# khwajamoiz01/cadence

Hardware: AMD Instinct MI355X
Metric: history events replayed/sec (node) + workflows rebuilt/sec; % HBM peak (higher is better)
Workload: dtype int64

## Files before the change

cadence_amd/csrc/replay_kernel.hip:

```cpp

#include <hip/hip_runtime.h>
#include <stddef.h>
#include <stdint.h>

#include <type_traits>
#include <utility>

#include "cadence_replay.h"

#ifndef CRR_LDS_ACT
#define CRR_LDS_ACT 2
#endif
#ifndef CRR_LDS_TIMER
#define CRR_LDS_TIMER 2
#endif
#ifndef CRR_LDS_CHILD
#define CRR_LDS_CHILD 1
#endif
#ifndef CRR_LDS_RC
#define CRR_LDS_RC 1
#endif
#ifndef CRR_LDS_SIG
#define CRR_LDS_SIG 1
#endif
// ... 2570 lines not shown
    i64 bt = 0, be = 0;
    if (cnt > CRR_WAVE_MIN_SCALAR) {
      i64 v = 0x7fffffffffffffffLL;
      each<N>([&](auto k) { v = (ok[k] && t[k] < v) ? t[k] : v; });
      const i64 wm = WaveTables<HbmRows>::wave_min_i64(v);
      each<N>([&](auto k) { m[k] = __builtin_amdgcn_ballot_w64(ok[k] && t[k] == wm); });
    }
    each<N>([&](auto k) {
      for (u64 x = m[k]; x; x &= x - 1) {
        const i32 l = (i32)__builtin_ctzll(x);
        const i64 tt = readlane_i64(t[k], l), ee = readlane_i64(id[k], l);
        if (best < 0 || tt < bt || (tt == bt && ee < be)) { best = 64 * k + l; bt = tt; be = ee; }
      }
    });
    tmin = bt;
    return best;
  }
  __device__ __forceinline__ void epilogue(Lane& L, const Geo& G, const TaskSink& K) {
    if (L.n_act > 0 && dirty_act) {
      u32 ok[NA];
      each<NA>([&](auto k) { ok[k] = (a_fl[k] & (kMirLive | kMirHave)) == (kMirLive | kMirHave); });
      i64 t = 0;
      const i32 j = argmin<NA>(ok, a_ct, a_id, t);
      if (j >= 0) {
        const u32 fl = get<NA>(a_fl, j);
        const i32 y = (i32)((fl >> 9) & 7u);
        if (!(fl & kMirCreated)) {
          set_bits<NA>(a_fl, j, kMirCreated | (timer_mask(y) << 16), 0u);
          if (y == CRR_TIMEOUT_HEARTBEAT) M->act[j].last_hb_timeout_vis_s = unix_seconds(t);
          if (K.on) K.add(L, G, CRR_TASK_ACTIVITY_TIMEOUT, y, L.current_version, t, get<NA>(a_id, j), M->act[j].attempt, -1);
        }
      }
    }
    dirty_act = false;
    if (L.n_timer > 0 && dirty_timer) {
      u32 ok[NT];
      each<NT>([&](auto k) { ok[k] = (t_fl[k] & kMirLive) != 0; });
      i64 t = 0;
      const i32 j = argmin<NT>(ok, t_ex, t_sid, t);
      if (j >= 0 && !(get<NT>(t_fl, j) & kMirTimerCreated)) {
        set_bits<NT>(t_fl, j, kMirTimerCreated, 0u);
        K.add(L, G, CRR_TASK_USER_TIMER, 0, L.current_version, t, get<NT>(t_sid, j), 0, -1);
      }
    }
    dirty_timer = false;
  }
  __device__ __forceinline__ void refresh(Lane& L, const Geo& G) {
    each<NA>([&](auto k) { a_fl[k] &= ~(kMirCreated | (0xffu << 16)); });
    each<NT>([&](auto k) { t_fl[k] &= ~kMirTimerCreated; });
    dirty_act = dirty_timer = true;
    epilogue(L, G, TaskSink{false, false});
  }

  template <int N, class Row, class Patch>
  __device__ __forceinline__ void scatter(const u32 (&fl)[N], const i64 (&id)[N], Row* rows, i64* ids,
                                          Row* (Geo::*dst)(i32) const, const Geo& G, Patch patch) const {
    i32 rank[N];
    u64 live[N];
    each<N>([&](auto k) { rank[k] = 0; live[k] = __builtin_amdgcn_ballot_w64((fl[k] & kMirLive) != 0); });
    each<N>([&](auto k2) {
      for (u64 x = live[k2]; x; x &= x - 1) {
        const i64 o = readlane_i64(id[k2], (i32)__builtin_ctzll(x));
        each<N>([&](auto k) { rank[k] += o < id[k] ? 1 : 0; });
      }
    });
    each<N>([&](auto k) {
      if ((fl[k] & kMirLive) != 0) {
        Row r = rows[64 * k + lane];
        patch(r, fl[k]);
        *(G.*dst)(rank[k]) = r;
        ids[rank[k]] = id[k];
      }
    });
  }
  __device__ __forceinline__ void finalize(Lane& L, const Geo& G) {
    i64* ids = M->ids;
    constexpr i32 oT = A, oC = oT + T, oR = oC + C, oS = oR + R;
    scatter<NA>(a_fl, a_id, M->act, ids, &Geo::act, G, [](crr_activity_row& r, u32 f) {
      r.flags = f & 0xffu;
      r.timer_task_status = (i32)((f >> 16) & 0xffu);
    });
    scatter<NT>(t_fl, t_sid, M->timer, ids + oT, &Geo::timer, G, [](crr_timer_row& r, u32 f) {
      r.flags = f & 0xffu;
      r.task_status = (f & kMirTimerCreated) ? CRR_TIMER_TASK_STATUS_CREATED : CRR_TIMER_TASK_STATUS_NONE;
    });
    scatter<NC>(c_fl, c_id, M->child, ids + oC, &Geo::child, G, [](crr_child_row& r, u32 f) { r.flags = f & 0xffu; });
    scatter<NR>(r_fl, r_id, M->rc, ids + oR, &Geo::rc, G, [](crr_initiated_row& r, u32 f) { r.flags = f & 0xffu; });
    scatter<NS>(s_fl, s_id, M->sig, ids + oS, &Geo::sig, G, [](crr_initiated_row& r, u32 f) { r.flags = f & 0xffu; });
    if (lane < L.n_rp) *G.rp(lane) = M->rp[lane];
    wave_sync_lds();
  }
  __device__ __forceinline__ i64 act_id(const Geo&, i32 i) const { return M->ids[i]; }
  __device__ __forceinline__ i64 timer_id(const Geo&, i32 i) const { return M->ids[A + i]; }
  __device__ __forceinline__ i64 child_id(const Geo&, i32 i) const { return M->ids[A + T + i]; }
  __device__ __forceinline__ i64 rc_id(const Geo&, i32 i) const { return M->ids[A + T + C + i]; }
  __device__ __forceinline__ i64 sig_id(const Geo&, i32 i) const { return M->ids[A + T + C + R + i]; }
  __device__ __forceinline__ void retry_push(const crr_inputs& in, const crr_outputs& out, u32 w) {
    retried = true;
    if constexpr (kList >= 0) {
      if (lane == 0) {
        const u32 k = atomicAdd(out.scratch + kList, 1u);
        out.scratch[retry_slot(in, kList, k)] = w;
      }
    }
  }
};

#if CRR_WAVE_REG
template <class ARENA, int LIST>
using WaveLds = WaveRegTables<ARENA, LIST>;
template <class ARENA, int LIST>
__device__ __forceinline__ void bind_arena(WaveRegTables<ARENA, LIST>& T, ARENA* a) { T.M = a; }
#else
template <class ARENA, int LIST>
using WaveLds = WaveTables<LdsRows<ARENA, LIST>>;
template <class ARENA, int LIST>
__device__ __forceinline__ void bind_arena(WaveTables<LdsRows<ARENA, LIST>>& T, ARENA* a) { T.S.M = a; }
#endif


namespace need {
constexpr u64 bit(int t) { return 1ull << t; }
constexpr u64 kTs = bit(CRR_EV_DECISION_TASK_SCHEDULED) | bit(CRR_EV_DECISION_TASK_STARTED) |
                    bit(CRR_EV_ACTIVITY_TASK_SCHEDULED) | bit(CRR_EV_ACTIVITY_TASK_STARTED) | bit(CRR_EV_TIMER_STARTED);
constexpr u64 kRef = bit(CRR_EV_DECISION_TASK_SCHEDULED) | bit(CRR_EV_DECISION_TASK_STARTED) |
                     bit(CRR_EV_DECISION_TASK_COMPLETED) | bit(CRR_EV_ACTIVITY_TASK_STARTED) |
                     bit(CRR_EV_ACTIVITY_TASK_COMPLETED) | bit(CRR_EV_ACTIVITY_TASK_FAILED) |
                     bit(CRR_EV_ACTIVITY_TASK_TIMED_OUT) | bit(CRR_EV_ACTIVITY_TASK_CANCELED) | bit(CRR_EV_TIMER_STARTED) |
                     bit(CRR_EV_START_CHILD_WORKFLOW_EXECUTION_FAILED) | bit(CRR_EV_CHILD_WORKFLOW_EXECUTION_STARTED) |
                     bit(CRR_EV_CHILD_WORKFLOW_EXECUTION_COMPLETED) | bit(CRR_EV_CHILD_WORKFLOW_EXECUTION_FAILED) |
                     bit(CRR_EV_CHILD_WORKFLOW_EXECUTION_CANCELED) | bit(CRR_EV_CHILD_WORKFLOW_EXECUTION_TIMED_OUT) |
                     bit(CRR_EV_CHILD_WORKFLOW_EXECUTION_TERMINATED) | bit(CRR_EV_REQUEST_CANCEL_EXTERNAL_FAILED) |
                     bit(CRR_EV_EXTERNAL_WORKFLOW_EXECUTION_CANCEL_REQUESTED) | bit(CRR_EV_SIGNAL_EXTERNAL_FAILED) |
                     bit(CRR_EV_EXTERNAL_WORKFLOW_EXECUTION_SIGNALED);
constexpr u64 kKey = bit(CRR_EV_DECISION_TASK_COMPLETED) | bit(CRR_EV_ACTIVITY_TASK_SCHEDULED) |
                     bit(CRR_EV_ACTIVITY_TASK_CANCEL_REQUESTED) | bit(CRR_EV_TIMER_STARTED) | bit(CRR_EV_TIMER_FIRED) |
                     bit(CRR_EV_TIMER_CANCELED);
constexpr u64 kAux = bit(CRR_EV_WORKFLOW_EXECUTION_STARTED) | bit(CRR_EV_DECISION_TASK_SCHEDULED) |
                     bit(CRR_EV_ACTIVITY_TASK_SCHEDULED) | bit(CRR_EV_REQUEST_CANCEL_EXTERNAL_INITIATED) |
                     bit(CRR_EV_WORKFLOW_EXECUTION_CONTINUED_AS_NEW) |
                     bit(CRR_EV_START_CHILD_WORKFLOW_EXECUTION_INITIATED) | bit(CRR_EV_SIGNAL_EXTERNAL_INITIATED);
constexpr u64 kTsTasks = bit(CRR_EV_WORKFLOW_EXECUTION_STARTED) | bit(CRR_EV_WORKFLOW_EXECUTION_COMPLETED) |
                         bit(CRR_EV_WORKFLOW_EXECUTION_FAILED) | bit(CRR_EV_WORKFLOW_EXECUTION_TIMED_OUT) |
                         bit(CRR_EV_WORKFLOW_EXECUTION_CANCELED) | bit(CRR_EV_WORKFLOW_EXECUTION_TERMINATED) |
                         bit(CRR_EV_WORKFLOW_EXECUTION_CONTINUED_AS_NEW);
__device__ __forceinline__ bool has(u64 mask, u32 et) { return (mask >> (et & CRR_ETYPE_MASK)) & 1ull; }
}

struct LaneSource {
  const crr_events& E;
  i64 begin, st;
  i32 n;
  Ev nx;
  u32 et_nx;
  u64 ts_mask;
  u64 aux_mask;
  __device__ __forceinline__ LaneSource(const crr_events& e, i64 b, i64 stride, i32 count, bool tasks, bool started_aux = false)
      : E(e), begin(b), st(stride), n(count), ts_mask(need::kTs | (tasks ? need::kTsTasks : 0ull)),
        aux_mask(need::kAux | (started_aux ? need::bit(CRR_EV_ACTIVITY_TASK_STARTED) : 0ull)) {}
  __device__ __forceinline__ i64 ix(i32 step) const { return begin + (i64)step * st; }
  __device__ __forceinline__ Ev load(i32 step, u32 et) const {
    Ev e;
    const i64 i = ix(step);
    e.et = et;
    e.id_ = E.event_id[i];
    e.ver_ = E.version[i];
    e.ts_ = need::has(ts_mask, et) ? E.timestamp[i] : 0;
    e.ref_ = need::has(need::kRef, et) ? E.ref[i] : 0;
    e.key_ = need::has(need::kKey, et) ? E.key[i] : 0u;
    e.aux_ = need::has(aux_mask, et) ? E.aux[i] : 0;
    e.task_ = 0;
    return e;
  }
  __device__ __forceinline__ void start() {
    if (n > 0) {
      const i64 i = ix(0);
      nx.et = E.etype[i];
      et_nx = E.etype[ix(n > 1 ? 1 : 0)];
      nx.id_ = E.event_id[i];
      nx.ver_ = E.version[i];
      nx.ts_ = E.timestamp[i];
      nx.ref_ = E.ref[i];
      nx.key_ = E.key[i];
      nx.aux_ = E.aux[i];
      nx.task_ = 0;
    }
  }
  __device__ __forceinline__ Ev next(i32 s) {
    const Ev e = nx;
    issue(s);
    return e;
  }
  __device__ __forceinline__ void issue(i32 s) {
    if (s + 1 < n) nx = load(s + 1, et_nx);
    if (s + 2 < n) et_nx = E.etype[ix(s + 2)];
  }
  __device__ __forceinline__ i64 task_id(i32 step) const { return E.task_id[ix(step)]; }
};

struct WaveLaneSource : LaneSource {
  i64 ubase;
  __device__ __forceinline__ WaveLaneSource(const crr_events& e, i64 b, i32 count, bool tasks)
      : LaneSource(e, b, 64, count, tasks), ubase(uniform64(b - (i64)threadIdx.x)) {}
  template <class T>
  __device__ __forceinline__ T at(const T* col, i32 step) const {
    static_assert(sizeof(T) == 1 || sizeof(T) == 4 || sizeof(T) == 8, "column width");
    const i64 row = uniform64((i64)reinterpret_cast<uintptr_t>(col + (ubase + (i64)step * 64)));
    u32 off;
    if constexpr (sizeof(T) == 1) asm("v_mov_b32 %0, %1 ; step %2" : "=v"(off) : "v"(threadIdx.x), "s"(step));
    else if constexpr (sizeof(T) == 4) asm("v_lshlrev_b32 %0, 2, %1 ; step %2" : "=v"(off) : "v"(threadIdx.x), "s"(step));
    else asm("v_lshlrev_b32 %0, 3, %1 ; step %2" : "=v"(off) : "v"(threadIdx.x), "s"(step));
    typedef const T __attribute__((address_space(1))) * global_ptr;
    return *(global_ptr)((u64)row + (u64)off);
  }
  __device__ __forceinline__ Ev load(i32 step, u32 et) const {
    Ev e;
    e.et = et;
    e.id_ = at(E.event_id, step);
    e.ver_ = at(E.version, step);
    e.ts_ = need::has(ts_mask, et) ? at(E.timestamp, step) : 0;
    e.ref_ = need::has(need::kRef, et) ? at(E.ref, step) : 0;
    e.key_ = need::has(need::kKey, et) ? at(E.key, step) : 0u;
    e.aux_ = need::has(aux_mask, et) ? at(E.aux, step) : 0;
    e.task_ = 0;
    return e;
  }
  __device__ __forceinline__ void start() {
    if (n > 0) {
      nx.et = at(E.etype, 0);
      et_nx = E.etype[ix(n > 1 ? 1 : 0)];
      nx.id_ = at(E.event_id, 0);
      nx.ver_ = at(E.version, 0);
      nx.ts_ = at(E.timestamp, 0);
      nx.ref_ = at(E.ref, 0);
      nx.key_ = at(E.key, 0);
      nx.aux_ = at(E.aux, 0);
      nx.task_ = 0;
    }
  }
  __device__ __forceinline__ Ev next(i32 s) {
    const Ev e = nx;
    issue(s);
    return e;
  }
  __device__ __forceinline__ void issue(i32 s) {
    const i32 su = uniform32(s);
    if (s + 1 < n) nx = load(su + 1, et_nx);
    if (s + 2 < n) et_nx = at(E.etype, su + 2);
  }
};

#ifndef CRR_WAVE_FIELDS
#define CRR_WAVE_FIELDS 1
#endif
struct WaveSource {
  const crr_events& E;
  i64 begin, st;
  i32 n, lane;
  Ev cur, nxt;
  __device__ __forceinline__ WaveSource(const crr_events& e, i64 b, i64 stride, i32 count)
      : E(e), begin(b), st(stride), n(uniform32(count)) {
    lane = (i32)(threadIdx.x & 63);
  }
  __device__ __forceinline__ Ev load_chunk(i32 c) const {
    Ev e;
    const i32 s = c * 64 + lane;
    const i64 ix = begin + (i64)(s < n ? s : 0) * st;
    e.et = E.etype[ix]; e.id_ = E.event_id[ix]; e.ver_ = E.version[ix]; e.ts_ = E.timestamp[ix];
    e.task_ = 0; e.ref_ = E.ref[ix]; e.key_ = E.key[ix]; e.aux_ = E.aux[ix];
    return e;
  }
  __device__ __forceinline__ i64 task_id(i32 step) const { return E.task_id[begin + (i64)step * st]; }
  __device__ __forceinline__ void start() {
    if (n > 0) cur = load_chunk(0);
  }
  __device__ __forceinline__ void rotate() { cur = nxt; }
  __device__ __forceinline__ void issue_next(i32 c) {
    if ((c + 1) * 64 < n) nxt = load_chunk(c + 1);
  }
};
__device__ __forceinline__ u32 lane_u32(u32 v, i32 l) {
#if CRR_WAVE_FIELDS == 0
  return (u32)__shfl((int)v, l, 64);
#else
  const u32 r = __builtin_amdgcn_readlane(v, l);
#if CRR_WAVE_FIELDS == 2
  u32 o;
  asm("v_mov_b32 %0, %1" : "=v"(o) : "s"(r));
  return o;
#else
  return r;
#endif
#endif
}
__device__ __forceinline__ i64 lane_i64(i64 v, i32 l) {
  const u32 lo = lane_u32((u32)(u64)v, l), hi = lane_u32((u32)((u64)v >> 32), l);
  return (i64)(((u64)hi << 32) | lo);
}
struct SidePf {
  i32 s2s, s2c, st2c, hb, retry, dom;
};
struct WaveEv {
  const Ev& C;
  i32 l;
  u32 et;
  const SidePf* sp;
  __device__ __forceinline__ crr_activity_side act_side(const crr_inputs&) const {
    crr_activity_side a{};
    a.schedule_to_start = (i32)lane_u32((u32)sp->s2s, l);
    a.schedule_to_close = (i32)lane_u32((u32)sp->s2c, l);
    a.start_to_close = (i32)lane_u32((u32)sp->st2c, l);
    a.heartbeat = (i32)lane_u32((u32)sp->hb, l);
    a.has_retry_policy = (i32)lane_u32((u32)sp->retry, l);
    a.domain_status = (i32)lane_u32((u32)sp->dom, l);
    return a;
  }
  __device__ __forceinline__ i64 id() const { return lane_i64(C.id_, l); }
  __device__ __forceinline__ i64 ver() const { return lane_i64(C.ver_, l); }
  __device__ __forceinline__ i64 ts() const { return lane_i64(C.ts_, l); }
  __device__ __forceinline__ i64 task() const { return 0; }
  __device__ __forceinline__ i64 ref() const { return lane_i64(C.ref_, l); }
  __device__ __forceinline__ u32 key() const { return lane_u32(C.key_, l); }
  __device__ __forceinline__ i32 aux() const { return (i32)lane_u32((u32)C.aux_, l); }
};

struct TokenDesc { u32 so, sl, fo, fl; };
__device__ __forceinline__ TokenDesc token_desc(const crr_workflow* wfp) {
  return TokenDesc{wfp->start_token_off, wfp->start_token_len, wfp->final_token_off, wfp->final_token_len};
}
struct TokenWords {
  static constexpr int kWords = 12;
  u64 w[kWords];
  u32 off, len, held;
  u32 raw;
  bool spliced;
  __device__ __forceinline__ void issue(const TokenDesc& d, i32 token_src, const uint8_t* arena,
                                        const uint32_t* token_crc = nullptr, u32 wi = 0) {
    off = 0; len = 0;
    if (token_src == 1) { off = d.so; len = d.sl; }
    if (token_src == 2) { off = d.fo; len = d.fl; }
    spliced = token_src == 1 && token_crc != nullptr && len == kSpliceBytes;
    raw = spliced ? token_crc[wi] : 0u;
    held = (off & 7u) || spliced ? 0u : (len & ~7u);
    held = held < 8u * kWords ? held : 8u * kWords;
    const u64* tw = reinterpret_cast<const u64*>(arena + off);
#pragma unroll
    for (int j = 0; j < kWords; ++j) w[j] = (8u * j + 8u <= held) ? tw[j] : 0ull;
  }
};

template <class IDS>
__device__ __forceinline__ u32 payload_crc(const crr_exec_row& R, const IDS& ids, const Geo& G, const TokenWords& TW,
                                           const uint8_t* arena, const u32* tables, u32* out_len,
                                           bool have_last = false, i64 last_id = 0, i64 last_ver = 0,
                                           int64_t* const* sink = nullptr, bool sink_writer = false) {
  Crc K;
  K.init(tables);
  K.u8(0x59);
  K.field(2, 10); K.u8((R.flags & CRR_EXEC_CANCEL_REQUESTED) ? 1 : 0);
  K.field(6, 15); K.be16((u32)(uint16_t)(int16_t)R.state);
  K.field(10, 23); K.be64(R.last_first_event_id);
  K.field(10, 24); K.be64(R.next_event_id);
  K.field(10, 25); K.be64(R.last_processed_event);
  K.field(10, 26); K.be64((i64)R.signal_count);
  K.field(8, 35); K.be32((u32)(i32)R.decision_attempt);
  K.field(10, 36); K.be64(R.decision_version);
  K.field(10, 37); K.be64(R.decision_schedule_id);
  K.field(10, 38); K.be64(R.decision_started_id);
  const bool sk = sink != nullptr && sink_writer;
  auto put = [&](int t, i64 base, i32 i, i64 id) {
    if (sk) sink[t][base + (i64)i * G.st] = id;
    K.be64(id);
  };
  K.list_header(45, 10, (u32)R.n_timer);
  for (i32 i = 0; i < R.n_timer; ++i) put(1, G.timer_base, i, ids.timer_id(G, i));
  K.list_header(46, 10, (u32)R.n_activity);
  for (i32 i = 0; i < R.n_activity; ++i) put(0, G.act_base, i, ids.act_id(G, i));
  K.list_header(47, 10, (u32)R.n_signal);
  for (i32 i = 0; i < R.n_signal; ++i) put(4, G.sig_base, i, ids.sig_id(G, i));
  K.list_header(48, 10, (u32)R.n_rc);
  for (i32 i = 0; i < R.n_rc; ++i) put(3, G.rc_base, i, ids.rc_id(G, i));
  K.list_header(49, 10, (u32)R.n_child);
  for (i32 i = 0; i < R.n_child; ++i) put(2, G.child_base, i, ids.child_id(G, i));
  K.field(11, 55); K.be32(0);
  K.field(12, 56);
  K.field(8, 10); K.be32(0);
  K.list_header(20, 12, 1u);
  const u32 tlen = TW.len;
  K.field(11, 10); K.be32(tlen);
  if (TW.spliced) {
    K.splice(TW.raw);
  } else {
#pragma unroll
    for (int j = 0; j < TokenWords::kWords; ++j)
      if (8u * j + 8u <= TW.held) K.push(TW.w[j], 8);
    const uint8_t* tp = arena + TW.off;
    u32 i = TW.held;
    if ((TW.off & 7u) == 0) {
      const u64* tw = reinterpret_cast<const u64*>(tp);
      for (; i + 8 <= tlen; i += 8) K.push(tw[i >> 3], 8);
    }
// ... 704 lines not shown
        const u64 seg = le(lane) & ~le(bl);
        const bool carried_dirty = T.dirty_act || T.dirty_timer;
        u64 RPV = 0;
        for (u64 rpm = RP; rpm;) {
          const i32 j = (i32)__builtin_ctzll(rpm);
          const u32 key = __builtin_amdgcn_readlane(C.key_, j);
          rpm &= ~__builtin_amdgcn_ballot_w64(live && is_dc && C.key_ == key);
          if (!T.rp_has(L, G, key)) RPV |= 1ull << j;
        }
        const u64 EB = __builtin_amdgcn_ballot_w64(live && (C.et & CRR_ETYPE_BATCH_LAST) &&
                                                   ((MP & seg) != 0 || (bl < 0 && carried_dirty)));
        OPS = MP | RPV;
        vm = (OPS | EB) & le(stop - 1);
      }
      const u64 BF = __builtin_amdgcn_ballot_w64(live && (C.et & CRR_ETYPE_BATCH_FIRST));
      constexpr u64 kBatchIdTypes = (1ull << CRR_EV_ACTIVITY_TASK_SCHEDULED) |
                                    (1ull << CRR_EV_START_CHILD_WORKFLOW_EXECUTION_INITIATED) |
                                    (1ull << CRR_EV_REQUEST_CANCEL_EXTERNAL_INITIATED) |
                                    (1ull << CRR_EV_SIGNAL_EXTERNAL_INITIATED);
      i32 wfail = -1;
      int wrc = CRR_OK;
      while (vm) {
        const i32 j = (i32)__builtin_ctzll(vm);
        vm &= vm - 1;
        const i32 s = c0 + j;
        const WaveEv ev{C, j, (u32)__builtin_amdgcn_readlane(C.et, j), &SP};
        const u32 et = ev.et;
        i64 bfid = batch_first_id;
        if (!fast) {
          if (et & CRR_ETYPE_BATCH_FIRST) batch_first_id = ev.id();
          bfid = batch_first_id;
          L.current_version = L.state == CRR_STATE_COMPLETED ? lane_i64(pver, j) : ev.ver();
          last_task_step = s;
        } else if (((1ull << (et & CRR_ETYPE_MASK)) & kBatchIdTypes) != 0) {
          const i32 bf = last_in(BF & le(j));
          if (bf >= 0) bfid = lane_i64(C.id_, bf);
        }
        if (!fast || ((OPS >> j) & 1)) {
          const int rc = uniform32(apply_event(in, out, L, G, T, ev, s + L.src_base, (i32)(et & CRR_ETYPE_MASK), bfid,
                                               now_ns, K, retention_days));
          if (rc) {
            wfail = j;
            wrc = rc;
            break;
          }
        }
        if (et & CRR_ETYPE_BATCH_LAST) {
          T.epilogue(L, G, K);
          if (!fast) {
            L.last_first_event_id = batch_first_id;
            L.next_event_id = ev.id() + 1;
          }
        }
      }
      if (fast) {
        const i32 end = wfail >= 0 ? wfail : stop;
        const i32 dend = (wfail >= 0 && (__builtin_amdgcn_readlane(tl, wfail) == CRR_EV_DECISION_TASK_COMPLETED)) ? wfail + 1 : end;
        const bool lv = live && lane < dend;
        const bool is_ds = tl == CRR_EV_DECISION_TASK_SCHEDULED, is_dt = tl == CRR_EV_DECISION_TASK_STARTED;
        const bool is_dc = tl == CRR_EV_DECISION_TASK_COMPLETED;
        const bool is_df = tl == CRR_EV_DECISION_TASK_TIMED_OUT || tl == CRR_EV_DECISION_TASK_FAILED;
        const u64 DM = __builtin_amdgcn_ballot_w64(lv && (is_ds || is_dt || is_dc || is_df));
        const u64 DS = __builtin_amdgcn_ballot_w64(lv && is_ds), DT = __builtin_amdgcn_ballot_w64(lv && is_dt);
        const u64 DC = __builtin_amdgcn_ballot_w64(lv && is_dc);
        const u64 BL = __builtin_amdgcn_ballot_w64(lv && (C.et & CRR_ETYPE_BATCH_LAST));
        const u64 E = le(end - 1);
        const i32 p = last_in(DM);
        if (p >= 0) {
          const i32 tp = (i32)__builtin_amdgcn_readlane(tl, p);
          auto att_at = [&](i32 x) -> i64 {
            const i32 v = last_in((DS | DT | DC) & le(x - 1));
            const i64 base = v < 0 ? L.decision_attempt : ((DS >> v) & 1) ? lane_i64(C.ref_, v) : 0;
            return base + __builtin_popcountll(DM & le(x) & ~le(v));
          };
          i64 nv, ns, nst = CRR_EMPTY_EVENT_ID, natt = 0, nsts = 0, nscts = 0, nots = 0;
          i32 nreq = CRR_SRC_EMPTY_UUID, nto = 0;
          if (tp == CRR_EV_DECISION_TASK_SCHEDULED) {
            nv = lane_i64(C.ver_, p); ns = lane_i64(C.id_, p); nto = (i32)lane_u32((u32)C.aux_, p);
            natt = lane_i64(C.ref_, p); nscts = lane_i64(C.ts_, p); nots = nscts;
          } else if (tp == CRR_EV_DECISION_TASK_STARTED || tp == CRR_EV_DECISION_TASK_COMPLETED) {
            const i32 r = last_in((DM & ~(DT | DC)) & le(p - 1));
            nots = r < 0 ? L.decision_orig_scheduled_ts : ((DS >> r) & 1) ? lane_i64(C.ts_, r) : 0;
            if (tp == CRR_EV_DECISION_TASK_STARTED) {
              const i32 q = last_in(DM & ~DT & le(p - 1));
              if (q < 0) {
                nto = L.decision_timeout;
                nscts = L.decision_scheduled_ts;
              } else if ((DS >> q) & 1) {
                nto = (i32)lane_u32((u32)C.aux_, q);
                nscts = lane_i64(C.ts_, q);
              } else if ((DC >> q) & 1) {
                nto = 0;
                nscts = 0;
              } else {
                nto = att_at(q) != 0 ? L.decision_start_to_close : 0;
                nscts = now_ns;
              }
              nv = lane_i64(C.ver_, p); ns = lane_i64(C.ref_, p); nst = lane_i64(C.id_, p);
              nreq = c0 + p + L.src_base; nsts = lane_i64(C.ts_, p);
            } else {
              nv = CRR_EMPTY_VERSION; ns = CRR_EMPTY_EVENT_ID;
            }
          } else {
            natt = att_at(p);
            const bool tr = natt != 0;
            const i32 b = last_in(BL & le(p - 1));
            nv = tr ? lane_i64(C.ver_, p) : (i64)CRR_EMPTY_VERSION;
            ns = !tr ? (i64)CRR_EMPTY_EVENT_ID : b < 0 ? L.next_event_id : lane_i64(C.id_, b) + 1;
            nto = tr ? L.decision_start_to_close : 0;
            nscts = now_ns;
          }
          update_decision(L, nv, ns, nst, nreq, nto, natt, nsts, nscts, nots);
        }
        const i32 q = last_in(DC);
        if (q >= 0) L.last_processed_event = lane_i64(C.ref_, q);
        if (DS & E) {
          L.state = CRR_STATE_RUNNING;
          L.close_status = CRR_CLOSE_NONE;
        }
        const u64 SG = __builtin_amdgcn_ballot_w64(lv && tl == CRR_EV_WORKFLOW_EXECUTION_SIGNALED);
        const u64 CR = __builtin_amdgcn_ballot_w64(lv && tl == CRR_EV_WORKFLOW_EXECUTION_CANCEL_REQUESTED);
        L.signal_count = (i32)((u32)L.signal_count + (u32)__builtin_popcountll(SG & E));
        if (CR & E) L.flags |= CRR_EXEC_CANCEL_REQUESTED;
        const i32 b = last_in(BL & E);
        if (b >= 0) {
          const i32 bf = last_in(BF & le(b));
          L.last_first_event_id = bf < 0 ? batch_first_id : lane_i64(C.id_, bf);
          L.next_event_id = lane_i64(C.id_, b) + 1;
        }
        const i32 f = last_in(BF & E);
        if (f >= 0) batch_first_id = lane_i64(C.id_, f);
        const i32 k = wfail >= 0 ? wfail : stop < lim ? stop : lim - 1;
        if (k >= 0) {
          L.current_version = lane_i64(C.ver_, k);
          last_task_step = c0 + k;
        }
        if (wfail < 0 && stop < lim) {
          wfail = stop;
          wrc = CRR_ERR_DECISION_NOT_FOUND;
        }
      }
      if (wfail >= 0) {
        WAVE_VH_AFTER(wfail);
        FAIL(wrc, c0 + wfail);
      }
      if (lim > 0) WAVE_VH_AFTER(lim - 1);
      if (lim < cnt) {
        if (__builtin_amdgcn_readlane((u32)rc0, lim) == 0)
          L.current_version = L.state == CRR_STATE_COMPLETED ? lane_i64(pver, lim) : lane_i64(C.ver_, lim);
        FAIL((i32)__builtin_amdgcn_readlane((u32)prc, lim), c0 + lim);
      }
#undef WAVE_VH_AFTER
    }
  } else
  for (i32 s = 0; s < n_ev; ++s) {
    const Ev ev = src.next(s);
    const u32 et = ev.et;
    const i64 id = ev.id();
    const i64 ver = ev.ver();
    const i32 t = et & CRR_ETYPE_MASK;
    if (et & CRR_ETYPE_BATCH_FIRST) batch_first_id = id;
    {
      const bool completed = L.state == CRR_STATE_COMPLETED;
      const bool first = L.vh_n == 0;
      const bool grow = !first && ver > L.vh_last_ver;
      i32 rc0 = s == empty_at ? (i32)CRR_ERR_EMPTY_HISTORY : (completed && first) ? (i32)CRR_ERR_VH_EMPTY : 0;
      if (rc0 == 0) L.current_version = completed ? L.vh_last_ver : ver;
      const i32 vh_rc = (id < 0 || (ver < 0 && ver != CRR_EMPTY_VERSION)) ? (i32)CRR_ERR_VH_INVALID_ITEM
                        : first ? (G.vh_cap < 1 ? (i32)CRR_ERR_CAPACITY : 0)
                        : ver < L.vh_last_ver ? (i32)CRR_ERR_VH_LOWER_VERSION
                        : id <= L.vh_last_id ? (i32)CRR_ERR_VH_EVENT_ID_NOT_INCREASING
                        : (grow && L.vh_n >= G.vh_cap) ? (i32)CRR_ERR_CAPACITY : 0;
      rc0 = rc0 ? rc0 : vh_rc;
      if (rc0) FAIL(rc0, s);
      if (grow) {
        crr_vh_item* it = G.vh(L.vh_n - 1);
        it->event_id = L.vh_last_id;
        it->version = L.vh_last_ver;
      }
      L.vh_n += (first || grow) ? 1 : 0;
      L.vh_last_id = id;
      L.vh_last_ver = ver;
    }
    last_task_step = s;

    {
      int rc;
      const i32 tu = uniform32(t);
      const i32 ps = s + L.src_base;
      if (__builtin_amdgcn_ballot_w64(t != tu) == 0)
        rc = apply_event(in, out, L, G, T, ev, ps, tu, batch_first_id, now_ns,
                         K, retention_days);
      else if (LaneDispatch<P>::value)
        rc = apply_event_lanes(in, out, L, G, T, ev, ps, t, batch_first_id,
                               now_ns, K, retention_days);
      else
        rc = apply_event(in, out, L, G, T, ev, ps, t, batch_first_id, now_ns,
                         K, retention_days);
      if (rc) FAIL(rc, s);
    }

    if (et & CRR_ETYPE_BATCH_LAST) {
      T.epilogue(L, G, K);
      L.last_first_event_id = batch_first_id;
      L.next_event_id = id + 1;
    }
  }
  {
    if (last_task_step >= 0) L.last_event_task_id = src.task_id(last_task_step);
    task_read = true;
    tok.so = wfp->start_token_off; tok.sl = wfp->start_token_len;
    tok.fo = wfp->final_token_off; tok.fl = wfp->final_token_len;
    const u32 final_len = tok.fl;
    const i64 want_id = wfp->rebuild_last_event_id, want_ver = wfp->rebuild_last_event_version;
    const u32 wf_flags = wfp->flags;
    if (empty_at == n_ev) FAIL(CRR_ERR_EMPTY_HISTORY, n_ev);
    if (final_len != 0xFFFFFFFFu) {
      L.token_src = 2;
      if (L.vh_n == 0) FAIL(CRR_ERR_VH_EMPTY, n_ev);
      if (want_id < 0 || (want_ver < 0 && want_ver != CRR_EMPTY_VERSION)) FAIL(CRR_ERR_VH_INVALID_ITEM, n_ev);
      if (L.vh_last_id != want_id || L.vh_last_ver != want_ver) FAIL(CRR_ERR_REBUILD_LAST_ITEM, n_ev);
    }
    if (wf_flags & CRR_WF_FLAG_REFRESH_TASKS) {
      L.n_tasks = 0;
      CHECK_N(refresh_tasks_head(in, L, G, K, src, n_ev, now_ns, retention_days));
      T.refresh(L, G);
    }
  }
done_events:
  CRR_PHASE(2);
#undef CHECK
#undef CHECK_N
#undef FAIL
  if (!task_read && last_task_step >= 0) L.last_event_task_id = src.task_id(last_task_step);

  if (L.status == CRR_OK && K.on && L.n_tasks > G.task_cap) L.status = CRR_ERR_CAPACITY;
  if (L.status == CRR_INTERNAL_RETRY) {
    if constexpr (BeforeRetry<P>::value) T.before_retry(L, G);
    out.exec[w].status = CRR_INTERNAL_RETRY;
    T.retry_push(in, out, w);
    return;
  }
  bool want_crc = L.status == CRR_OK;
  TokenWords TW;
  TW.issue(tok, want_crc ? L.token_src : 0, in.arena, in.token_crc, w);
  u64 dkey = 0;
  if (dg && digest_ptr()) dkey = digest_keys_ptr()[w];
  if constexpr (std::is_same<SRC, WaveSource>::value) wave_sync_global();
  if (L.vh_n > 0) {
    crr_vh_item* it = G.vh(L.vh_n - 1);
    it->event_id = L.vh_last_id;
    it->version = L.vh_last_ver;
  }
  CRR_PHASE(3);
  T.finalize(L, G);
  CRR_PHASE(4);
  if constexpr (EMIT) {
    if (K.on && want_crc && (wfp->flags & CRR_WF_FLAG_REFRESH_TASKS)) {
      if constexpr (std::is_same<SRC, WaveSource>::value) wave_sync_global();
      refresh_tasks_rows(in, L, G, K);
      if (L.n_tasks > G.task_cap) {
        L.status = CRR_ERR_CAPACITY;
        L.fail_step = n_ev + L.src_base;
        want_crc = false;
      }
    }
  }

  crr_exec_row R;
  R.status = L.status;
  R.fail_step = L.fail_step;
  R.inconsistencies = L.inconsistencies;
  R.flags = L.flags | (L.status == CRR_OK ? CRR_EXEC_CHECKSUM_VALID : 0u);
  R.state = L.state;
  R.close_status = L.close_status;
  R.signal_count = L.signal_count;
  R.decision_timeout = L.decision_timeout;
  R.next_event_id = L.next_event_id;
  R.last_first_event_id = L.last_first_event_id;
  R.last_event_task_id = L.last_event_task_id;
  R.last_processed_event = L.last_processed_event;
  R.completion_event_batch_id = L.completion_event_batch_id;
  R.decision_version = L.decision_version;
  R.decision_schedule_id = L.decision_schedule_id;
  R.decision_started_id = L.decision_started_id;
  R.decision_attempt = L.decision_attempt;
  R.decision_started_ts = L.decision_started_ts;
  R.decision_scheduled_ts = L.decision_scheduled_ts;
  R.decision_orig_scheduled_ts = L.decision_orig_scheduled_ts;
  R.current_version = L.current_version;
  R.decision_request_src = L.decision_request_src;
  R.start_src = L.start_src;
  R.n_activity = L.n_act;
  R.n_timer = L.n_timer;
  R.n_child = L.n_child;
  R.n_rc = L.n_rc;
  R.n_signal = L.n_sig;
  R.n_vh_items = L.vh_n;
  R.n_reset_points = L.n_rp;
  R.token_src = L.token_src;
  R.checksum = 0;
  R.payload_len = 0;
  R.n_tasks = L.n_tasks;
  R.decision_start_to_close = L.decision_start_to_close;
  R.expiration_ns = L.expiration_ns;
  R.src_next = L.src_base + n_ev;
  R.reserved = 0;
  if (want_crc) {
    int64_t* const* sink = out.live_ids[0] ? out.live_ids : nullptr;
    R.checksum = payload_crc(R, T, G, TW, in.arena, crc_tables, &R.payload_len, true, L.vh_last_id, L.vh_last_ver, sink,
                             !std::is_same<SRC, WaveSource>::value || (threadIdx.x & 63) == 0);
  }
  CRR_PHASE(5);
  out.exec[w] = R;
  if (dg && digest_ptr() && (!std::is_same<SRC, WaveSource>::value || (threadIdx.x & 63) == 0))
    dg->add(R, n_ev, dkey);
#if CRR_PHASE_PROF
  if constexpr (!std::is_same<SRC, WaveSource>::value) {
    if ((wfp->flags & CRR_WF_FLAG_RESUME) && (threadIdx.x & 63) == 0 && ph[1] != 0) {
      atomicAdd(&g_phase_prof[0], ph[1] - ph[0]);
      atomicAdd(&g_phase_prof[1], ph[2] - ph[1]);
      atomicAdd(&g_phase_prof[2], ph[3] - ph[2]);
      atomicAdd(&g_phase_prof[3], ph[4] - ph[3]);
      atomicAdd(&g_phase_prof[4], ph[5] - ph[4]);
      atomicAdd(&g_phase_prof[5], 1ull);
    }
  }
#endif
}
#if CRR_PHASE_PROF
extern "C" int crr_phase_prof(unsigned long long* host, int reset) {
  if (hipMemcpyFromSymbol(host, HIP_SYMBOL(g_phase_prof), sizeof(g_phase_prof)) != hipSuccess) return -1;
  if (reset) {
    unsigned long long z[8] = {};
    if (hipMemcpyToSymbol(HIP_SYMBOL(g_phase_prof), z, sizeof(z)) != hipSuccess) return -1;
  }
  return 0;
}
#endif

__device__ __forceinline__ u32 lane_count(const crr_inputs& in) {
  return (in.flags & CRR_IN_WAVE_TAIL) ? in.wave_begin : in.n_wf;
}
__device__ __forceinline__ u32 tail_count_end(const crr_inputs& in) {
  return ((in.flags & CRR_IN_TIERED) && in.big_begin >= in.wave_begin && in.big_begin < in.n_wf) ? in.big_begin : in.n_wf;
}
__device__ __forceinline__ i64 wf_stride(const crr_inputs& in, u32 w) {
  return ((in.flags & CRR_IN_WAVE_TAIL) && w >= in.wave_begin) ? 1 : (i64)in.stride;
}

#ifndef CRR_SMALL_CRC
#define CRR_SMALL_CRC 0
#endif
template <class TIER> struct WaveTier;
template <> struct WaveTier<SmallTier> { using Arena = WaveArena<40, 32, 16, 8, 8, 24>; };
template <> struct WaveTier<LargeTier> { using Arena = WaveArena<64, 48, 24, 16, 16, 32>; };
template <class TIER>
union BlockArena {
  LdsArena<TIER> lane;
// ... 438 lines not shown
```

Before: 71.95 billion.

## Double-buffer event prefetch in per-lane replay loop with ping-pong registers

Measured after the change: 71.04 billion. 0.987x the previous value.

```diff
diff --git a/cadence_amd/csrc/replay_kernel.hip b/cadence_amd/csrc/replay_kernel.hip
--- a/cadence_amd/csrc/replay_kernel.hip
+++ b/cadence_amd/csrc/replay_kernel.hip
@@ -2746,6 +2746,7 @@
   i64 begin, st;
   i32 n;
   Ev nx;
+  Ev ny;
   u32 et_nx;
   u64 ts_mask;
   u64 aux_mask;
@@ -2780,13 +2781,14 @@
       nx.task_ = 0;
     }
   }
-  __device__ __forceinline__ Ev next(i32 s) {
-    const Ev e = nx;
-    issue(s);
-    return e;
-  }
+  template <bool ODD>
+  __device__ __forceinline__ void arrived() const {
+    const Ev& e = ODD ? ny : nx;
+    asm volatile("" ::"v"(e.id_), "v"(e.ver_), "v"(e.ts_), "v"(e.ref_), "v"(e.key_), "v"(e.aux_), "v"(et_nx) : "memory");
+  }
+  template <bool ODD>
   __device__ __forceinline__ void issue(i32 s) {
-    if (s + 1 < n) nx = load(s + 1, et_nx);
+    if (s + 1 < n) (ODD ? ny : nx) = load(s + 1, et_nx);
     if (s + 2 < n) et_nx = E.etype[ix(s + 2)];
   }
   __device__ __forceinline__ i64 task_id(i32 step) const { return E.task_id[ix(step)]; }
@@ -2832,15 +2834,12 @@
       nx.task_ = 0;
     }
   }
-  __device__ __forceinline__ Ev next(i32 s) {
-    const Ev e = nx;
-    issue(s);
-    return e;
-  }
+  template <bool ODD>
   __device__ __forceinline__ void issue(i32 s) {
     const i32 su = uniform32(s);
-    if (s + 1 < n) nx = load(su + 1, et_nx);
+    const u32 et1 = et_nx;
     if (s + 2 < n) et_nx = at(E.etype, su + 2);
+    if (s + 1 < n) (ODD ? ny : nx) = load(su + 1, et1);
   }
 };
 
@@ -3851,15 +3850,14 @@
       }
 #undef WAVE_VH_AFTER
     }
-  } else
-  for (i32 s = 0; s < n_ev; ++s) {
-    const Ev ev = src.next(s);
-    const u32 et = ev.et;
-    const i64 id = ev.id();
-    const i64 ver = ev.ver();
-    const i32 t = et & CRR_ETYPE_MASK;
-    if (et & CRR_ETYPE_BATCH_FIRST) batch_first_id = id;
-    {
+  } else {
+    bool failed = false;
+    auto step = [&](const Ev& ev, const i32 s) __attribute__((always_inline)) {
+      const u32 et = ev.et;
+      const i64 id = ev.id();
+      const i64 ver = ev.ver();
+      const i32 t = et & CRR_ETYPE_MASK;
+      if (et & CRR_ETYPE_BATCH_FIRST) batch_first_id = id;
       const bool completed = L.state == CRR_STATE_COMPLETED;
       const bool first = L.vh_n == 0;
       const bool grow = !first && ver > L.vh_last_ver;
@@ -3870,40 +3868,52 @@
                         : ver < L.vh_last_ver ? (i32)CRR_ERR_VH_LOWER_VERSION
                         : id <= L.vh_last_id ? (i32)CRR_ERR_VH_EVENT_ID_NOT_INCREASING
                         : (grow && L.vh_n >= G.vh_cap) ? (i32)CRR_ERR_CAPACITY : 0;
-      rc0 = rc0 ? rc0 : vh_rc;
-      if (rc0) FAIL(rc0, s);
-      if (grow) {
-        crr_vh_item* it = G.vh(L.vh_n - 1);
-        it->event_id = L.vh_last_id;
-        it->version = L.vh_last_ver;
-      }
-      L.vh_n += (first || grow) ? 1 : 0;
-      L.vh_last_id = id;
-      L.vh_last_ver = ver;
-    }
-    last_task_step = s;
-
-    {
-      int rc;
-      const i32 tu = uniform32(t);
-      const i32 ps = s + L.src_base;
-      if (__builtin_amdgcn_ballot_w64(t != tu) == 0)
-        rc = apply_event(in, out, L, G, T, ev, ps, tu, batch_first_id, now_ns,
-                         K, retention_days);
-      else if (LaneDispatch<P>::value)
-        rc = apply_event_lanes(in, out, L, G, T, ev, ps, t, batch_first_id,
-                               now_ns, K, retention_days);
-      else
-        rc = apply_event(in, out, L, G, T, ev, ps, t, batch_first_id, now_ns,
-                         K, retention_days);
-      if (rc) FAIL(rc, s);
-    }
-
-    if (et & CRR_ETYPE_BATCH_LAST) {
-      T.epilogue(L, G, K);
-      L.last_first_event_id = batch_first_id;
-      L.next_event_id = id + 1;
-    }
+      int rc = rc0 ? rc0 : vh_rc;
+      if (rc == 0) {
+        if (grow) {
+          crr_vh_item* it = G.vh(L.vh_n - 1);
+          it->event_id = L.vh_last_id;
+          it->version = L.vh_last_ver;
+        }
+        L.vh_n += (first || grow) ? 1 : 0;
+        L.vh_last_id = id;
+        L.vh_last_ver = ver;
+        last_task_step = s;
+
+        const i32 tu = uniform32(t);
+        const i32 ps = s + L.src_base;
+        if (__builtin_amdgcn_ballot_w64(t != tu) == 0)
+          rc = apply_event(in, out, L, G, T, ev, ps, tu, batch_first_id, now_ns,
+                           K, retention_days);
+        else if (LaneDispatch<P>::value)
+          rc = apply_event_lanes(in, out, L, G, T, ev, ps, t, batch_first_id,
+                                 now_ns, K, retention_days);
+        else
+          rc = apply_event(in, out, L, G, T, ev, ps, t, batch_first_id, now_ns,
+                           K, retention_days);
+        if (rc == 0 && (et & CRR_ETYPE_BATCH_LAST)) {
+          T.epilogue(L, G, K);
+          L.last_first_event_id = batch_first_id;
+          L.next_event_id = id + 1;
+        }
+      }
+      asm("; step status %0" : "+v"(rc));
+      L.status = rc;
+      L.fail_step = rc ? s + L.src_base : L.fail_step;
+      failed = rc != 0;
+    };
+    static_assert(CRR_OK == 0, "the latched status of a step that passed is CRR_OK");
+    for (i32 s = 0; s < n_ev && !failed; s += 2) {
+      src.template arrived<false>();
+      src.template issue<true>(s);
+      step(src.nx, s);
+      if (!failed && s + 1 < n_ev) {
+        src.template arrived<true>();
+        src.template issue<false>(s + 1);
+        step(src.ny, s + 1);
+      }
+    }
+    if (failed) goto done_events;
   }
   {
     if (last_task_step >= 0) L.last_event_task_id = src.task_id(last_task_step);
```
